# caishiqing/voice-tts

Measured on AMD Instinct MI355X. Metric: audio_seconds_per_second, higher is better.
Workload: dtype bf16

## Files before the change

### voice-tts_amd/csrc/gemm_x6.hip

```cpp
#include "common.h"

namespace ixtts {

typedef float gx_f32x16 __attribute__((ext_vector_type(16)));
typedef __bf16 gx_bf16x8 __attribute__((ext_vector_type(8)));
typedef float gx_f32x4 __attribute__((ext_vector_type(4)));
typedef unsigned int gx_u32x4 __attribute__((ext_vector_type(4)));


__global__ void gemm_x6_pack_kernel(const float* __restrict__ w, uint4* __restrict__ out, int N, int K, int Npad) {
  const long total = (long)(K / 8) * Npad;
  for (long idx = blockIdx.x * (long)blockDim.x + threadIdx.x; idx < total; idx += (long)gridDim.x * blockDim.x) {
    const int n = (int)(idx % Npad);
    const int ko = (int)(idx / Npad);
    float v[8];
#pragma unroll
    for (int e = 0; e < 8; ++e) v[e] = n < N ? w[(long)n * K + ko * 8 + e] : 0.f;
    uint4 ph, pm, pl;
    split8_bf16x3(v, ph, pm, pl);
    const int g = ko >> 1, kh = ko & 1;
    uint4* base = out + ((long)g * 6) * Npad + n;
    base[(long)(0 * 2 + kh) * Npad] = ph;
    base[(long)(1 * 2 + kh) * Npad] = pm;
    base[(long)(2 * 2 + kh) * Npad] = pl;
  }
}

template <int HALO>
__device__ __forceinline__ long split_src_row(long rr, int hT, int hleft, int hright, const int* __restrict__ hoff, int hn) {
  if constexpr (HALO == 0) return rr;
  long o0;
  int T = hT;
  if constexpr (HALO == 1) {
    o0 = rr / (hleft + hT + hright) * (hleft + hT + hright);
  } else {
    const int s = seq_of_row(hoff, hn, rr);
    o0 = hoff[s];
    T = hoff[s + 1] - (int)o0 - hleft - hright;
    if (T <= hleft || T <= hright) return rr;
  }
  const int h = (int)(rr - o0);
  if (h < hleft) return o0 + 2 * hleft - h;
  if (h >= hleft + T && h < hleft + T + hright) return o0 + 2 * (hleft + T) - 2 - h;
  return rr;
}

template <int HALO = 0>
__global__ __launch_bounds__(256) void gemm_x6_split_kernel(const float* __restrict__ a, long lda, uint4* __restrict__ out, int M, int K, long Mpad, int hT = 0,
                                                            int hleft = 0, int hright = 0, const int* __restrict__ hoff = nullptr, int hn = 0) {
  __shared__ float tile[64][65];
  const int r0 = blockIdx.x * 64, k0 = blockIdx.y * 64;
  const int t = threadIdx.x;
#pragma unroll
  for (int i = 0; i < 4; ++i) {
    const int r = (t >> 4) + 16 * i, kq = t & 15;
    float4 v = make_float4(0.f, 0.f, 0.f, 0.f);
    if (r0 + r < M) v = *reinterpret_cast<const float4*>(a + split_src_row<HALO>(r0 + r, hT, hleft, hright, hoff, hn) * lda + k0 + 4 * kq);
    tile[r][4 * kq + 0] = v.x; tile[r][4 * kq + 1] = v.y; tile[r][4 * kq + 2] = v.z; tile[r][4 * kq + 3] = v.w;
  }
  __syncthreads();
#pragma unroll
  for (int u = 0; u < 2; ++u) {
    const int r = t & 63, o = (t >> 6) + 4 * u;
    float v[8];
#pragma unroll
    for (int e = 0; e < 8; ++e) v[e] = tile[r][o * 8 + e];
    uint4 ph, pm, pl;
    split8_bf16x3(v, ph, pm, pl);
    const int ko = (k0 >> 3) + o, g = ko >> 1, kh = ko & 1;
    uint4* base = out + ((long)g * 6) * Mpad + r0 + r;
    base[(long)(0 * 2 + kh) * Mpad] = ph;
    base[(long)(1 * 2 + kh) * Mpad] = pm;
    base[(long)(2 * 2 + kh) * Mpad] = pl;
  }
}

enum { EPI_PLAIN = 0, EPI_SWIGLU = 1, EPI_GATE = 2 };

struct GemmX6Params {
  const uint4* Ap;
  long Mpad;
  long arow0;
  const uint4* Wp;
  const float* bias;
  float* C;
  long ldc;
  int M, N, Npad, K, accumulate, m_tiles, n_tiles;
  int tap_steps;
  int epi;
  const float* gate;
  long gate_ld, rows_per_batch;
  int nbatch;
  const int* gate_seq_off;
  unsigned long long* dbg;
};


template <int MT, int NT, int NST, int EPI = EPI_PLAIN, int ACC = 0, int SEQ = 0, int DBG = 0, int PIN = 0>
__global__ __launch_bounds__(256, (NST * (MT + NT) * 6 * 64 * 16 <= 80 * 1024) ? 2 : 1) void gemm_x6_kernel(GemmX6Params p) {
  constexpr int BM = 64 * MT, BN = 64 * NT;
  constexpr int A_UNITS = 6 * BM, W_UNITS = 6 * BN, STAGE = A_UNITS + W_UNITS;
  constexpr int NDMA = (6 * (MT + NT)) / 4;
  constexpr int NA = (6 * MT) / 4, NW = NDMA - NA;
  static_assert((6 * MT) % 4 == 0 && (6 * NT) % 4 == 0, "the A pieces and the W pieces are each dealt evenly to the 4 waves");
  static_assert(EPI == EPI_PLAIN || (ACC == 0 && NT == 2), "pair epilogues: the wave's two 32-column blocks are the two halves");
  static_assert(EPI == EPI_GATE || SEQ == 0, "the sequence table belongs to the gate epilogue");
  constexpr int D = NST - 1;
  extern __shared__ uint4 smem[];

  const int nwg = p.m_tiles * p.n_tiles;
  const int bid = blockIdx.x;
  const int xcd = bid & 7, idx = bid >> 3;
  const int qd = nwg >> 3, rm = nwg & 7;
  const int lin = (xcd < rm ? xcd * (qd + 1) : rm * (qd + 1) + (xcd - rm) * qd) + idx;
  const int m_tile = lin / p.n_tiles, n_tile = lin - m_tile * p.n_tiles;
  const int m0 = m_tile * BM, n0 = n_tile * BN;

  const int tid = threadIdx.x, lane = tid & 63;
  const int wave = __builtin_amdgcn_readfirstlane(tid >> 6);
  const int wm = wave >> 1, wn = wave & 1;
  const int l31 = lane & 31, lh = lane >> 5;

  gx_f32x16 acc[MT][NT];
#pragma unroll
  for (int i = 0; i < MT; ++i)
#pragma unroll
    for (int j = 0; j < NT; ++j)
#pragma unroll
      for (int r = 0; r < 16; ++r) acc[i][j][r] = 0.f;

  const uint4* asrc = p.Ap + p.arow0 + m0 + lane;
  const uint4* wsrc = p.Wp + n0 + lane;
  long a_off[NA], w_off[NW];
  int a_lds[NA], w_lds[NW];
#pragma unroll
  for (int q = 0; q < NA; ++q) {
    const int e = q * 4 + wave, run = e / MT, piece = e % MT;
    a_off[q] = run * p.Mpad + piece * 64;
    a_lds[q] = run * BM + piece * 64;
  }
#pragma unroll
  for (int q = 0; q < NW; ++q) {
    const int e = q * 4 + wave, run = e / NT, piece = e % NT;
    w_off[q] = (long)run * p.Npad + piece * 64;
    w_lds[q] = A_UNITS + run * BN + piece * 64;
  }
  const long a_step = 6 * p.Mpad, w_step = 6L * p.Npad;
  const long a_wrap = 1 - p.tap_steps * a_step;
  long a_run = 0, w_run = 0;
  int a_group = 0;
  auto issue_next = [&](uint4* st) {
#pragma unroll
    for (int q = 0; q < NA; ++q)
      __builtin_amdgcn_global_load_lds((const __attribute__((address_space(1))) void*)(asrc + (a_off[q] + a_run)),
                                       (__attribute__((address_space(3))) void*)(st + a_lds[q]), 16, 0, 0);
#pragma unroll
    for (int q = 0; q < NW; ++q)
      __builtin_amdgcn_global_load_lds((const __attribute__((address_space(1))) void*)(wsrc + (w_off[q] + w_run)),
                                       (__attribute__((address_space(3))) void*)(st + w_lds[q]), 16, 0, 0);
    a_run += a_step;
    w_run += w_step;
    if (++a_group == p.tap_steps) {
      a_group = 0;
      a_run += a_wrap;
    }
  };

  const int steps = p.K >> 4;
  auto wg_stamp = [&](int k) {
    if constexpr (DBG == 3) {
      if (tid == 0) p.dbg[128 + (long)blockIdx.x * 4 + k] = __builtin_amdgcn_s_memrealtime();
    }
  };
  auto wait_younger = [&](int y) {
    if (y >= 2) asm volatile("s_waitcnt vmcnt(%0)" ::"n"(2 * NDMA) : "memory");
    else if (y == 1) asm volatile("s_waitcnt vmcnt(%0)" ::"n"(NDMA) : "memory");
    else asm volatile("s_waitcnt vmcnt(0)" ::: "memory");
  };
  static_assert(D >= 1 && D <= 3, "1..3 steps of copies in flight behind the one waited for");
  wg_stamp(0);
  for (int t = 0; t < D && t < steps; ++t) issue_next(smem + t * STAGE);
  wait_younger(min(D, steps) - 1);
  __builtin_amdgcn_s_barrier();
  asm volatile("" ::: "memory");
  wg_stamp(1);

  const unsigned base_addr = (unsigned)(uintptr_t)(const __attribute__((address_space(3))) void*)smem;
  int st_cur = 0, st_nxt = D % NST;
  for (int s = 0; s < steps; ++s) {
    auto stamp = [&](int k) {
      if constexpr (DBG == 3) {
        if (blockIdx.x == 0 && tid == 0 && s < 16) {
          p.dbg[s * 8 + k] = __builtin_amdgcn_s_memtime();
          if (k == 0) p.dbg[s * 8 + 7] = __builtin_amdgcn_s_memrealtime();
        }
      }
    };
    stamp(0);
    if (DBG != 1 && s + D < steps) issue_next(smem + st_nxt * STAGE);
    stamp(1);
    const unsigned cur_addr = base_addr + (unsigned)(st_cur * STAGE * 16);
    if constexpr (DBG != 2) {
      gx_u32x4 af[3][MT], bf[3][NT];
      const unsigned aaddr = cur_addr + (unsigned)((lh * BM + wm * (32 * MT) + l31) * 16);
      const unsigned waddr = cur_addr + (unsigned)((A_UNITS + lh * BN + wn * (32 * NT) + l31) * 16);
      if constexpr (MT == 4 && NT == 2) {
        asm volatile(
            "ds_read_b128 %0, %18 offset:%20\n ds_read_b128 %1, %18 offset:%21\n ds_read_b128 %2, %18 offset:%22\n ds_read_b128 %3, %18 offset:%23\n"
            "ds_read_b128 %4, %18 offset:%24\n ds_read_b128 %5, %18 offset:%25\n ds_read_b128 %6, %18 offset:%26\n ds_read_b128 %7, %18 offset:%27\n"
            "ds_read_b128 %8, %18 offset:%28\n ds_read_b128 %9, %18 offset:%29\n ds_read_b128 %10, %18 offset:%30\n ds_read_b128 %11, %18 offset:%31\n"
            "ds_read_b128 %12, %19 offset:%32\n ds_read_b128 %13, %19 offset:%33\n ds_read_b128 %14, %19 offset:%34\n ds_read_b128 %15, %19 offset:%35\n"
            "ds_read_b128 %16, %19 offset:%36\n ds_read_b128 %17, %19 offset:%37\n s_waitcnt lgkmcnt(0)"
            : "=&v"(af[0][0]), "=&v"(af[0][1]), "=&v"(af[0][2]), "=&v"(af[0][3]), "=&v"(af[1][0]), "=&v"(af[1][1]), "=&v"(af[1][2]), "=&v"(af[1][3]),
              "=&v"(af[2][0]), "=&v"(af[2][1]), "=&v"(af[2][2]), "=&v"(af[2][3]), "=&v"(bf[0][0]), "=&v"(bf[0][1]), "=&v"(bf[1][0]), "=&v"(bf[1][1]),
              "=&v"(bf[2][0]), "=&v"(bf[2][1])
            : "v"(aaddr), "v"(waddr), "n"((0 * 2 * BM + 0) * 16), "n"((0 * 2 * BM + 32) * 16), "n"((0 * 2 * BM + 64) * 16), "n"((0 * 2 * BM + 96) * 16),
              "n"((1 * 2 * BM + 0) * 16), "n"((1 * 2 * BM + 32) * 16), "n"((1 * 2 * BM + 64) * 16), "n"((1 * 2 * BM + 96) * 16), "n"((2 * 2 * BM + 0) * 16),
              "n"((2 * 2 * BM + 32) * 16), "n"((2 * 2 * BM + 64) * 16), "n"((2 * 2 * BM + 96) * 16), "n"((0 * 2 * BN + 0) * 16), "n"((0 * 2 * BN + 32) * 16),
              "n"((1 * 2 * BN + 0) * 16), "n"((1 * 2 * BN + 32) * 16), "n"((2 * 2 * BN + 0) * 16), "n"((2 * 2 * BN + 32) * 16)
            : "memory");
      } else {
        static_assert(MT == 2 && NT == 2, "fragment block written for 256 x 128 and 128 x 128 tiles");
        asm volatile(
            "ds_read_b128 %0, %12 offset:%14\n ds_read_b128 %1, %12 offset:%15\n ds_read_b128 %2, %12 offset:%16\n ds_read_b128 %3, %12 offset:%17\n"
            "ds_read_b128 %4, %12 offset:%18\n ds_read_b128 %5, %12 offset:%19\n ds_read_b128 %6, %13 offset:%20\n ds_read_b128 %7, %13 offset:%21\n"
            "ds_read_b128 %8, %13 offset:%22\n ds_read_b128 %9, %13 offset:%23\n ds_read_b128 %10, %13 offset:%24\n ds_read_b128 %11, %13 offset:%25\n"
            "s_waitcnt lgkmcnt(0)"
            : "=&v"(af[0][0]), "=&v"(af[0][1]), "=&v"(af[1][0]), "=&v"(af[1][1]), "=&v"(af[2][0]), "=&v"(af[2][1]), "=&v"(bf[0][0]), "=&v"(bf[0][1]),
              "=&v"(bf[1][0]), "=&v"(bf[1][1]), "=&v"(bf[2][0]), "=&v"(bf[2][1])
            : "v"(aaddr), "v"(waddr), "n"((0 * 2 * BM + 0) * 16), "n"((0 * 2 * BM + 32) * 16), "n"((1 * 2 * BM + 0) * 16), "n"((1 * 2 * BM + 32) * 16),
              "n"((2 * 2 * BM + 0) * 16), "n"((2 * 2 * BM + 32) * 16), "n"((0 * 2 * BN + 0) * 16), "n"((0 * 2 * BN + 32) * 16), "n"((1 * 2 * BN + 0) * 16),
              "n"((1 * 2 * BN + 32) * 16), "n"((2 * 2 * BN + 0) * 16), "n"((2 * 2 * BN + 32) * 16)
            : "memory");
      }
      stamp(2);
#pragma unroll
      for (int i = 0; i < MT; ++i)
#pragma unroll
        for (int j = 0; j < NT; ++j) {
          const gx_bf16x8 ah = __builtin_bit_cast(gx_bf16x8, af[0][i]), am = __builtin_bit_cast(gx_bf16x8, af[1][i]), al = __builtin_bit_cast(gx_bf16x8, af[2][i]);
          const gx_bf16x8 bh = __builtin_bit_cast(gx_bf16x8, bf[0][j]), bm = __builtin_bit_cast(gx_bf16x8, bf[1][j]), bl = __builtin_bit_cast(gx_bf16x8, bf[2][j]);
          acc[i][j] = __builtin_amdgcn_mfma_f32_32x32x16_bf16(al, bh, acc[i][j], 0, 0, 0);
          acc[i][j] = __builtin_amdgcn_mfma_f32_32x32x16_bf16(ah, bl, acc[i][j], 0, 0, 0);
          acc[i][j] = __builtin_amdgcn_mfma_f32_32x32x16_bf16(am, bm, acc[i][j], 0, 0, 0);
          acc[i][j] = __builtin_amdgcn_mfma_f32_32x32x16_bf16(am, bh, acc[i][j], 0, 0, 0);
          acc[i][j] = __builtin_amdgcn_mfma_f32_32x32x16_bf16(ah, bm, acc[i][j], 0, 0, 0);
          acc[i][j] = __builtin_amdgcn_mfma_f32_32x32x16_bf16(ah, bh, acc[i][j], 0, 0, 0);
        }
      if constexpr (DBG == 3) asm volatile("" ::"v"(acc[0][0][0]), "v"(acc[MT - 1][NT - 1][15]));
      if constexpr (PIN != 0) __builtin_amdgcn_sched_barrier(0);
    }
    stamp(3);
    wait_younger(DBG == 1 ? 0 : max(0, min(D - 1, steps - s - 2)));
    stamp(4);
    __builtin_amdgcn_s_barrier();
    asm volatile("" ::: "memory");
    stamp(5);
    st_cur = st_cur + 1 == NST ? 0 : st_cur + 1;
    st_nxt = st_nxt + 1 == NST ? 0 : st_nxt + 1;
  }

  wg_stamp(2);
  if constexpr (EPI != EPI_PLAIN) {
    const int oc = (n0 + wn * 64) / 2 + l31;
    const int nh = p.N >> 1;
    if (oc < nh) {
      const unsigned rpb = (unsigned)min(p.rows_per_batch, (long)0x7fffffff);
      const float ba = p.bias != nullptr ? p.bias[n0 + wn * 64 + l31] : 0.f, bb = p.bias != nullptr ? p.bias[n0 + wn * 64 + 32 + l31] : 0.f;
#pragma unroll
      for (int i = 0; i < MT; ++i) {
        const int rbase = m0 + wm * (32 * MT) + i * 32 + 4 * lh;
#pragma unroll
        for (int r = 0; r < 16; ++r) {
          const int row = rbase + (r & 3) + 8 * (r >> 2);
          if (row < p.M) {
            float a = acc[i][0][r] + ba, b = acc[i][1][r] + bb, v;
            if constexpr (EPI == EPI_SWIGLU) {
              v = a / (1.0f + expf(-a)) * b;
            } else {
              long gb;
              if constexpr (SEQ != 0) gb = (long)seq_of_row(p.gate_seq_off, p.nbatch, row);
              else gb = min((long)((unsigned)row / rpb), (long)p.nbatch - 1);
              const float* g = p.gate + gb * p.gate_ld;
              a += g[oc];
              b += g[nh + oc];
              v = tanhf(a) * (1.0f / (1.0f + expf(-b)));
            }
            p.C[(long)row * p.ldc + oc] = v;
          }
        }
      }
    }
  } else
#pragma unroll
  for (int j = 0; j < NT; ++j) {
    const int col = n0 + wn * (32 * NT) + j * 32 + l31;
    const bool col_ok = col < p.N;
    const float bv = (p.bias != nullptr && col_ok) ? p.bias[col] : 0.f;
#pragma unroll
    for (int i = 0; i < MT; ++i) {
      const int rbase = m0 + wm * (32 * MT) + i * 32 + 4 * lh;
#pragma unroll
      for (int r = 0; r < 16; ++r) {
        const int row = rbase + (r & 3) + 8 * (r >> 2);
        if (col_ok && row < p.M) {
          float* c = p.C + (long)row * p.ldc + col;
          float v = acc[i][j][r] + bv;
          if constexpr (ACC != 0) v += *c;
          *c = v;
        }
      }
    }
  }
  if constexpr (DBG == 3) {
    asm volatile("s_waitcnt vmcnt(0)" ::: "memory");
    wg_stamp(3);
  }
}

template <int MT, int NT, int NST, int EPI = EPI_PLAIN, int ACC = 0, int SEQ = 0, int DBG = 0, int PIN = 0>
static int launch_gemm_x6(GemmX6Params p, hipStream_t st) {
  constexpr int BM = 64 * MT, BN = 64 * NT;
  constexpr size_t smem = (size_t)NST * (6 * BM + 6 * BN) * 16;
  static_assert(smem <= 160 * 1024, "LDS stages of this tile shape");
  p.m_tiles = ceil_div(p.M, BM);
  p.n_tiles = ceil_div(p.N, BN);
  IX_ARG((long)p.n_tiles * BN <= p.Npad, "gemm_x6: packed weights padded to %d features, the %d-wide tile needs %d", p.Npad, BN, p.n_tiles * BN);
  const int taps = (p.K >> 4) / p.tap_steps;
  IX_ARG(p.arow0 + (long)p.m_tiles * BM + taps - 1 <= p.Mpad, "gemm_x6: activation planes hold %ld rows, the %d-row tiles reach row %ld", p.Mpad, BM,
         p.arow0 + (long)p.m_tiles * BM + taps - 1);
  auto kern = gemm_x6_kernel<MT, NT, NST, EPI, ACC, SEQ, DBG, PIN>;
  static bool done = false;
  if (!done) {
    IX_HIP(hipFuncSetAttribute((const void*)kern, hipFuncAttributeMaxDynamicSharedMemorySize, (int)smem));
    done = true;
  }
  hipLaunchKernelGGL(kern, dim3(p.m_tiles * p.n_tiles), dim3(256), smem, st, p);
  IX_HIP(hipGetLastError());
  return IXTTS_OK;
}

template <int MT, int NT, int NST, bool PAIR>
static int launch_gemm_x6_epilogue(const GemmX6Params& p, hipStream_t st) {
  if (p.epi == EPI_PLAIN) return p.accumulate ? launch_gemm_x6<MT, NT, NST, EPI_PLAIN, 1>(p, st) : launch_gemm_x6<MT, NT, NST, EPI_PLAIN, 0>(p, st);
  if constexpr (PAIR) {
    if (p.epi == EPI_SWIGLU) return launch_gemm_x6<MT, NT, NST, EPI_SWIGLU>(p, st);
    if (p.epi == EPI_GATE)
      return p.gate_seq_off ? launch_gemm_x6<MT, NT, NST, EPI_GATE, 0, 1>(p, st) : launch_gemm_x6<MT, NT, NST, EPI_GATE, 0, 0>(p, st);
  }
  set_error("gemm_x6: epilogue %d on a tile shape built without it", p.epi);
  return IXTTS_ERR_ARG;
}

}

using namespace ixtts;

extern "C" size_t ixtts_gemm_x6_packed_bytes(int N, int K) {
  if (N <= 0 || K <= 0 || K % 64) return 0;
  const size_t Npad = (size_t)(N + 255) / 256 * 256;
  return (size_t)(K / 16) * 6 * Npad * 16;
}

extern "C" int ixtts_gemm_x6_pack(const float* w_dev, void* packed_dev, int N, int K, void* stream) {
  IX_ARG(w_dev && packed_dev && N > 0 && K > 0 && K % 64 == 0, "gemm_x6_pack: bad argument (K must be a multiple of 64)");
  const int Npad = (N + 255) / 256 * 256;
  const long total = (long)(K / 8) * Npad;
  hipLaunchKernelGGL(gemm_x6_pack_kernel, dim3((unsigned)std::min<long>((total + 255) / 256, 4096)), dim3(256), 0, (hipStream_t)stream, w_dev,
                     reinterpret_cast<uint4*>(packed_dev), N, K, Npad);
  IX_HIP(hipGetLastError());
  return IXTTS_OK;
}

extern "C" long ixtts_gemm_x6_rows_padded(long rows) { return rows <= 0 ? 0 : (rows + 255) / 256 * 256 + 256; }

extern "C" int ixtts_gemm_x6_split(const float* a_dev, long lda, void* planes_dev, long rows, int K, void* stream) {
  IX_ARG(a_dev && planes_dev && rows > 0 && K > 0 && K % 64 == 0, "gemm_x6_split: bad argument (K must be a multiple of 64)");
  IX_ARG(lda >= K && lda % 4 == 0 && (reinterpret_cast<uintptr_t>(a_dev) & 15) == 0, "gemm_x6_split: rows must be 16-byte aligned (lda %ld)", lda);
  const long Mpad = ixtts_gemm_x6_rows_padded(rows);
  hipLaunchKernelGGL(gemm_x6_split_kernel<0>, dim3((unsigned)(Mpad / 64), K / 64), dim3(256), 0, (hipStream_t)stream, a_dev, lda,
                     reinterpret_cast<uint4*>(planes_dev), (int)rows, K, Mpad);
  IX_HIP(hipGetLastError());
  return IXTTS_OK;
}

extern "C" int ixtts_gemm_x6_split_halo(const float* a_dev, long lda, void* planes_dev, long rows, int K, int T, int left, int right, void* stream) {
  IX_ARG(a_dev && planes_dev && rows > 0 && K > 0 && K % 64 == 0, "gemm_x6_split_halo: bad argument (K must be a multiple of 64)");
  IX_ARG(lda >= K && lda % 4 == 0 && (reinterpret_cast<uintptr_t>(a_dev) & 15) == 0, "gemm_x6_split_halo: rows must be 16-byte aligned (lda %ld)", lda);
  IX_ARG(left >= 0 && right >= 0 && T > left && T > right && rows % (left + T + right) == 0,
         "gemm_x6_split_halo: bad shape rows=%ld T=%d left=%d right=%d (rows = whole sequences of left + T + right)", rows, T, left, right);
  const long Mpad = ixtts_gemm_x6_rows_padded(rows);
  hipLaunchKernelGGL(gemm_x6_split_kernel<1>, dim3((unsigned)(Mpad / 64), K / 64), dim3(256), 0, (hipStream_t)stream, a_dev, lda,
                     reinterpret_cast<uint4*>(planes_dev), (int)rows, K, Mpad, T, left, right);
  IX_HIP(hipGetLastError());
  return IXTTS_OK;
}

extern "C" int ixtts_gemm_x6_split_halo_varlen(const float* a_dev, long lda, void* planes_dev, long rows, int K, const int* seq_off_dev, int nseq, int left,
                                               int right, void* stream) {
  IX_ARG(a_dev && planes_dev && seq_off_dev && rows > 0 && K > 0 && K % 64 == 0, "gemm_x6_split_halo_varlen: bad argument (K must be a multiple of 64)");
  IX_ARG(lda >= K && lda % 4 == 0 && (reinterpret_cast<uintptr_t>(a_dev) & 15) == 0, "gemm_x6_split_halo_varlen: rows must be 16-byte aligned (lda %ld)", lda);
  IX_ARG(nseq > 0 && left >= 0 && right >= 0, "gemm_x6_split_halo_varlen: bad shape nseq=%d left=%d right=%d", nseq, left, right);
  const long Mpad = ixtts_gemm_x6_rows_padded(rows);
  hipLaunchKernelGGL(gemm_x6_split_kernel<2>, dim3((unsigned)(Mpad / 64), K / 64), dim3(256), 0, (hipStream_t)stream, a_dev, lda,
                     reinterpret_cast<uint4*>(planes_dev), (int)rows, K, Mpad, 0, left, right, seq_off_dev, nseq);
  IX_HIP(hipGetLastError());
  return IXTTS_OK;
}

static int run_gemm_x6(GemmX6Params p, int tile, hipStream_t st) {
  if (tile == 0) {
    const long t42 = (long)ceil_div(p.M, 256) * ceil_div(p.N, 128);
    tile = t42 >= 140 ? 2 : 3;
  }
  switch (tile) {
    case 2: return launch_gemm_x6_epilogue<4, 2, 2, true>(p, st);
    case 3: return launch_gemm_x6_epilogue<2, 2, 3, true>(p, st);
    case 4: return launch_gemm_x6_epilogue<4, 2, 4, false>(p, st);
    case 5: return launch_gemm_x6_epilogue<2, 2, 4, false>(p, st);
  }
  if (tile >= 12 && (p.epi != EPI_PLAIN || p.accumulate)) {
    set_error("gemm_x6: the developer variants (tile %d) are built with the plain, overwriting epilogue only", tile);
    return IXTTS_ERR_ARG;
  }
  switch (tile) {
    case 12: return launch_gemm_x6<4, 2, 2, EPI_PLAIN, 0, 0, 1>(p, st);
    case 22: return launch_gemm_x6<4, 2, 2, EPI_PLAIN, 0, 0, 2>(p, st);
    case 32: return launch_gemm_x6<4, 2, 2, EPI_PLAIN, 0, 0, 3>(p, st);
    case 33: return launch_gemm_x6<2, 2, 3, EPI_PLAIN, 0, 0, 3>(p, st);
    case 42: return launch_gemm_x6<4, 2, 2, EPI_PLAIN, 0, 0, 0, 1>(p, st);
    case 43: return launch_gemm_x6<2, 2, 3, EPI_PLAIN, 0, 0, 0, 1>(p, st);
  }
  set_error("gemm_x6: tile %d (0 auto; 2 / 3: 256x128 / 128x128, two workgroups per CU; 4 / 5: the same, one per CU with a 4-stage ring)", tile);
  return IXTTS_ERR_ARG;
}

extern "C" int ixtts_gemm_x6_f32(const void* a_planes_dev, long rows_total, long row0, const void* packed_dev, const float* bias_dev, float* c_dev,
                                 long ldc, int M, int N, int K, int accumulate, int tile, void* stream) {
  IX_ARG(a_planes_dev && packed_dev && c_dev && M > 0 && N > 0 && K > 0 && K % 64 == 0, "gemm_x6: bad argument (K must be a multiple of 64: the split pass works on 64-wide k blocks)");
  IX_ARG(ldc >= N && row0 >= 0 && row0 + M <= rows_total, "gemm_x6: rows [%ld, %ld) of %ld, ldc %ld", row0, row0 + M, rows_total, ldc);
  GemmX6Params p;
  p.Ap = reinterpret_cast<const uint4*>(a_planes_dev); p.Mpad = ixtts_gemm_x6_rows_padded(rows_total); p.arow0 = row0;
  p.Wp = reinterpret_cast<const uint4*>(packed_dev); p.bias = bias_dev; p.C = c_dev; p.ldc = ldc;
  p.M = M; p.N = N; p.Npad = (N + 255) / 256 * 256; p.K = K; p.accumulate = accumulate ? 1 : 0; p.m_tiles = p.n_tiles = 0;
  p.tap_steps = K >> 4; p.epi = EPI_PLAIN; p.gate = nullptr; p.gate_ld = 0; p.rows_per_batch = 1; p.nbatch = 1; p.gate_seq_off = nullptr;
  p.dbg = (tile == 32 || tile == 33) ? reinterpret_cast<unsigned long long*>(const_cast<float*>(bias_dev)) : nullptr;
  if (p.dbg) p.bias = nullptr;
  return run_gemm_x6(p, tile, (hipStream_t)stream);
}

extern "C" int ixtts_gemm_x6_pair_f32(const void* a_planes_dev, long rows_total, long row0, int taps, const void* packed_dev, const float* bias_dev,
                                      const float* gate_dev, long gate_ld, long rows_per_batch, int nbatch, float* c_dev, long ldc, int M, int N, int K,
                                      int epilogue, int tile, void* stream) {
  IX_ARG(a_planes_dev && packed_dev && c_dev && M > 0 && N > 0 && taps > 0 && K > 0, "gemm_x6_pair: bad argument");
  IX_ARG(K % taps == 0 && (K / taps) % 64 == 0 && N % 64 == 0, "gemm_x6_pair: K %d = %d taps of a multiple of 64, N %d a multiple of 64", K, taps, N);
  IX_ARG(epilogue == EPI_SWIGLU || (epilogue == EPI_GATE && gate_dev && rows_per_batch > 0 && nbatch > 0 && gate_ld >= N / 2),
         "gemm_x6_pair: epilogue %d (1 swiglu; 2 gate, with gate biases)", epilogue);
  IX_ARG(ldc >= N / 2 && row0 >= 0 && row0 + M + taps - 1 <= rows_total, "gemm_x6_pair: rows [%ld, %ld) + %d taps of %ld, ldc %ld", row0, row0 + M, taps,
         rows_total, ldc);
  IX_ARG(tile == 0 || tile == 2 || tile == 3, "gemm_x6_pair: tile %d (0 auto, 2, 3)", tile);
  GemmX6Params p;
  p.Ap = reinterpret_cast<const uint4*>(a_planes_dev); p.Mpad = ixtts_gemm_x6_rows_padded(rows_total); p.arow0 = row0;
  p.Wp = reinterpret_cast<const uint4*>(packed_dev); p.bias = bias_dev; p.C = c_dev; p.ldc = ldc;
  p.M = M; p.N = N; p.Npad = (N + 255) / 256 * 256; p.K = K; p.accumulate = 0; p.m_tiles = p.n_tiles = 0;
  p.tap_steps = (K / taps) >> 4; p.epi = epilogue; p.gate = gate_dev; p.gate_ld = gate_ld; p.rows_per_batch = rows_per_batch; p.nbatch = nbatch;
  p.gate_seq_off = nullptr;
  p.dbg = nullptr;
  return run_gemm_x6(p, tile, (hipStream_t)stream);
}

extern "C" int ixtts_gemm_x6_pair_gate_varlen_f32(const void* a_planes_dev, long rows_total, long row0, int taps, const void* packed_dev, const float* bias_dev,
                                                  const float* gate_dev, long gate_ld, const int* seq_off_dev, int nseq, float* c_dev, long ldc, int M, int N,
                                                  int K, int tile, void* stream) {
  IX_ARG(seq_off_dev && nseq > 0, "gemm_x6_pair_gate_varlen: null offsets table or nseq %d", nseq);
  IX_ARG(a_planes_dev && packed_dev && c_dev && gate_dev && M > 0 && N > 0 && taps > 0 && K > 0 && gate_ld >= N / 2, "gemm_x6_pair_gate_varlen: bad argument");
  IX_ARG(K % taps == 0 && (K / taps) % 64 == 0 && N % 64 == 0, "gemm_x6_pair_gate_varlen: K %d = %d taps of a multiple of 64, N %d a multiple of 64", K, taps, N);
  IX_ARG(ldc >= N / 2 && row0 >= 0 && row0 + M + taps - 1 <= rows_total, "gemm_x6_pair_gate_varlen: rows [%ld, %ld) + %d taps of %ld, ldc %ld", row0, row0 + M,
         taps, rows_total, ldc);
  IX_ARG(tile == 0 || tile == 2 || tile == 3, "gemm_x6_pair_gate_varlen: tile %d (0 auto, 2, 3)", tile);
  GemmX6Params p;
  p.Ap = reinterpret_cast<const uint4*>(a_planes_dev); p.Mpad = ixtts_gemm_x6_rows_padded(rows_total); p.arow0 = row0;
  p.Wp = reinterpret_cast<const uint4*>(packed_dev); p.bias = bias_dev; p.C = c_dev; p.ldc = ldc;
  p.M = M; p.N = N; p.Npad = (N + 255) / 256 * 256; p.K = K; p.accumulate = 0; p.m_tiles = p.n_tiles = 0;
  p.tap_steps = (K / taps) >> 4; p.epi = EPI_GATE; p.gate = gate_dev; p.gate_ld = gate_ld; p.rows_per_batch = 1; p.nbatch = nseq;
  p.gate_seq_off = seq_off_dev;
  p.dbg = nullptr;
  return run_gemm_x6(p, tile, (hipStream_t)stream);
}
```

Measured before the change: 41.73.

## Add software-pipelined 128x128 gemm_x6 loop interleaving LDS reads and copies with MFMAs

Adds a PIPE variant of the 6-MFMA split-bf16 GEMM kernel for 128x128 tiles with a 4-stage ring. It double-buffers register fragments so the next step's LDS reads and the global-to-LDS copies are issued among the current step's MFMAs, pinned in place with sched_barriers. The auto tile selection uses this variant when the 128x128 grid fits within the CU count, aiming to hide LDS and global latency in small, latency-bound GEMMs. The cost is more registers, one workgroup per CU, and a K%64 requirement.

```diff
diff --git a/voice-tts_amd/csrc/gemm_x6.hip b/voice-tts_amd/csrc/gemm_x6.hip
--- a/voice-tts_amd/csrc/gemm_x6.hip
+++ b/voice-tts_amd/csrc/gemm_x6.hip
@@ -96,7 +96,7 @@
 };
 
 
-template <int MT, int NT, int NST, int EPI = EPI_PLAIN, int ACC = 0, int SEQ = 0, int DBG = 0, int PIN = 0>
+template <int MT, int NT, int NST, int EPI = EPI_PLAIN, int ACC = 0, int SEQ = 0, int DBG = 0, int PIN = 0, int PIPE = 0>
 __global__ __launch_bounds__(256, (NST * (MT + NT) * 6 * 64 * 16 <= 80 * 1024) ? 2 : 1) void gemm_x6_kernel(GemmX6Params p) {
   constexpr int BM = 64 * MT, BN = 64 * NT;
   constexpr int A_UNITS = 6 * BM, W_UNITS = 6 * BN, STAGE = A_UNITS + W_UNITS;
@@ -149,21 +149,26 @@
   const long a_wrap = 1 - p.tap_steps * a_step;
   long a_run = 0, w_run = 0;
   int a_group = 0;
-  auto issue_next = [&](uint4* st) {
-#pragma unroll
-    for (int q = 0; q < NA; ++q)
+  auto issue_piece = [&](uint4* st, int q) {
+    if (q < NA)
       __builtin_amdgcn_global_load_lds((const __attribute__((address_space(1))) void*)(asrc + (a_off[q] + a_run)),
                                        (__attribute__((address_space(3))) void*)(st + a_lds[q]), 16, 0, 0);
-#pragma unroll
-    for (int q = 0; q < NW; ++q)
-      __builtin_amdgcn_global_load_lds((const __attribute__((address_space(1))) void*)(wsrc + (w_off[q] + w_run)),
-                                       (__attribute__((address_space(3))) void*)(st + w_lds[q]), 16, 0, 0);
+    else
+      __builtin_amdgcn_global_load_lds((const __attribute__((address_space(1))) void*)(wsrc + (w_off[q - NA] + w_run)),
+                                       (__attribute__((address_space(3))) void*)(st + w_lds[q - NA]), 16, 0, 0);
+  };
+  auto issue_advance = [&]() {
     a_run += a_step;
     w_run += w_step;
     if (++a_group == p.tap_steps) {
       a_group = 0;
       a_run += a_wrap;
     }
+  };
+  auto issue_next = [&](uint4* st) {
+#pragma unroll
+    for (int q = 0; q < NDMA; ++q) issue_piece(st, q);
+    issue_advance();
   };
 
   const int steps = p.K >> 4;
@@ -179,16 +184,35 @@
   };
   static_assert(D >= 1 && D <= 3, "1..3 steps of copies in flight behind the one waited for");
   wg_stamp(0);
-  for (int t = 0; t < D && t < steps; ++t) issue_next(smem + t * STAGE);
-  wait_younger(min(D, steps) - 1);
-  __builtin_amdgcn_s_barrier();
-  asm volatile("" ::: "memory");
-  wg_stamp(1);
-
-  const unsigned base_addr = (unsigned)(uintptr_t)(const __attribute__((address_space(3))) void*)smem;
-  int st_cur = 0, st_nxt = D % NST;
-  for (int s = 0; s < steps; ++s) {
-    auto stamp = [&](int k) {
+  if constexpr (PIPE != 0) {
+    static_assert(MT == 2 && NT == 2 && NST == 4 && PIN == 0 && (DBG == 0 || DBG == 3), "the pipelined loop: 128 x 128 tile, 4 stages");
+    static_assert(D % NST != 0 && D % NST != 1 % NST && D % NST != 2 % NST, "(b): the copy target is none of the stages of steps s, s + 1, s + 2");
+    constexpr int RD_AT = 1, CP_AT = 2, CP_EVERY = 3;
+    static_assert(RD_AT < CP_AT && CP_AT + (NDMA - 1) * CP_EVERY < 6 * MT * NT, "reads, then the copies, all among the step's MFMAs");
+    const unsigned base_addr = (unsigned)(uintptr_t)(const __attribute__((address_space(3))) void*)smem;
+    const unsigned a_rel = (unsigned)((lh * BM + wm * (32 * MT) + l31) * 16), w_rel = (unsigned)((A_UNITS + lh * BN + wn * (32 * NT) + l31) * 16);
+    gx_u32x4 fa[2][3][MT], fb[2][3][NT];
+    auto read_issue = [&](gx_u32x4 (&a)[3][MT], gx_u32x4 (&b)[3][NT], int stage) {
+      const unsigned aaddr = base_addr + (unsigned)(stage * STAGE * 16) + a_rel, waddr = base_addr + (unsigned)(stage * STAGE * 16) + w_rel;
+      asm volatile(
+          "ds_read_b128 %0, %12 offset:%14\n ds_read_b128 %1, %12 offset:%15\n ds_read_b128 %2, %12 offset:%16\n ds_read_b128 %3, %12 offset:%17\n"
+          "ds_read_b128 %4, %12 offset:%18\n ds_read_b128 %5, %12 offset:%19\n ds_read_b128 %6, %13 offset:%20\n ds_read_b128 %7, %13 offset:%21\n"
+          "ds_read_b128 %8, %13 offset:%22\n ds_read_b128 %9, %13 offset:%23\n ds_read_b128 %10, %13 offset:%24\n ds_read_b128 %11, %13 offset:%25"
+          : "=&v"(a[0][0]), "=&v"(a[0][1]), "=&v"(a[1][0]), "=&v"(a[1][1]), "=&v"(a[2][0]), "=&v"(a[2][1]), "=&v"(b[0][0]),
+            "=&v"(b[0][1]), "=&v"(b[1][0]), "=&v"(b[1][1]), "=&v"(b[2][0]), "=&v"(b[2][1])
+          : "v"(aaddr), "v"(waddr), "n"((0 * 2 * BM + 0) * 16), "n"((0 * 2 * BM + 32) * 16), "n"((1 * 2 * BM + 0) * 16), "n"((1 * 2 * BM + 32) * 16),
+            "n"((2 * 2 * BM + 0) * 16), "n"((2 * 2 * BM + 32) * 16), "n"((0 * 2 * BN + 0) * 16), "n"((0 * 2 * BN + 32) * 16), "n"((1 * 2 * BN + 0) * 16),
+            "n"((1 * 2 * BN + 32) * 16), "n"((2 * 2 * BN + 0) * 16), "n"((2 * 2 * BN + 32) * 16)
+          : "memory");
+    };
+    auto read_wait = [&](gx_u32x4 (&a)[3][MT], gx_u32x4 (&b)[3][NT]) {
+      asm volatile("s_waitcnt lgkmcnt(0)"
+                   : "+v"(a[0][0]), "+v"(a[0][1]), "+v"(a[1][0]), "+v"(a[1][1]), "+v"(a[2][0]), "+v"(a[2][1]), "+v"(b[0][0]),
+                     "+v"(b[0][1]), "+v"(b[1][0]), "+v"(b[1][1]), "+v"(b[2][0]), "+v"(b[2][1])
+                   :
+                   : "memory");
+    };
+    auto stamp = [&](int s, int k) {
       if constexpr (DBG == 3) {
         if (blockIdx.x == 0 && tid == 0 && s < 16) {
           p.dbg[s * 8 + k] = __builtin_amdgcn_s_memtime();
@@ -196,68 +220,166 @@
         }
       }
     };
-    stamp(0);
-    if (DBG != 1 && s + D < steps) issue_next(smem + st_nxt * STAGE);
-    stamp(1);
-    const unsigned cur_addr = base_addr + (unsigned)(st_cur * STAGE * 16);
-    if constexpr (DBG != 2) {
-      gx_u32x4 af[3][MT], bf[3][NT];
-      const unsigned aaddr = cur_addr + (unsigned)((lh * BM + wm * (32 * MT) + l31) * 16);
-      const unsigned waddr = cur_addr + (unsigned)((A_UNITS + lh * BN + wn * (32 * NT) + l31) * 16);
-      if constexpr (MT == 4 && NT == 2) {
-        asm volatile(
-            "ds_read_b128 %0, %18 offset:%20\n ds_read_b128 %1, %18 offset:%21\n ds_read_b128 %2, %18 offset:%22\n ds_read_b128 %3, %18 offset:%23\n"
-            "ds_read_b128 %4, %18 offset:%24\n ds_read_b128 %5, %18 offset:%25\n ds_read_b128 %6, %18 offset:%26\n ds_read_b128 %7, %18 offset:%27\n"
-            "ds_read_b128 %8, %18 offset:%28\n ds_read_b128 %9, %18 offset:%29\n ds_read_b128 %10, %18 offset:%30\n ds_read_b128 %11, %18 offset:%31\n"
-            "ds_read_b128 %12, %19 offset:%32\n ds_read_b128 %13, %19 offset:%33\n ds_read_b128 %14, %19 offset:%34\n ds_read_b128 %15, %19 offset:%35\n"
-            "ds_read_b128 %16, %19 offset:%36\n ds_read_b128 %17, %19 offset:%37\n s_waitcnt lgkmcnt(0)"
-            : "=&v"(af[0][0]), "=&v"(af[0][1]), "=&v"(af[0][2]), "=&v"(af[0][3]), "=&v"(af[1][0]), "=&v"(af[1][1]), "=&v"(af[1][2]), "=&v"(af[1][3]),
-              "=&v"(af[2][0]), "=&v"(af[2][1]), "=&v"(af[2][2]), "=&v"(af[2][3]), "=&v"(bf[0][0]), "=&v"(bf[0][1]), "=&v"(bf[1][0]), "=&v"(bf[1][1]),
-              "=&v"(bf[2][0]), "=&v"(bf[2][1])
-            : "v"(aaddr), "v"(waddr), "n"((0 * 2 * BM + 0) * 16), "n"((0 * 2 * BM + 32) * 16), "n"((0 * 2 * BM + 64) * 16), "n"((0 * 2 * BM + 96) * 16),
-              "n"((1 * 2 * BM + 0) * 16), "n"((1 * 2 * BM + 32) * 16), "n"((1 * 2 * BM + 64) * 16), "n"((1 * 2 * BM + 96) * 16), "n"((2 * 2 * BM + 0) * 16),
-              "n"((2 * 2 * BM + 32) * 16), "n"((2 * 2 * BM + 64) * 16), "n"((2 * 2 * BM + 96) * 16), "n"((0 * 2 * BN + 0) * 16), "n"((0 * 2 * BN + 32) * 16),
-              "n"((1 * 2 * BN + 0) * 16), "n"((1 * 2 * BN + 32) * 16), "n"((2 * 2 * BN + 0) * 16), "n"((2 * 2 * BN + 32) * 16)
-            : "memory");
+    int st_rd = 1, st_cp = D % NST;
+    auto step = [&](auto set, auto copy, auto read, auto sync, int s) {
+      constexpr int c = decltype(set)::value;
+      constexpr bool COPY = decltype(copy)::value, READ = decltype(read)::value, SYNC = decltype(sync)::value;
+      static_assert(READ || !COPY, "copies are only issued for steps that will be read");
+      static_assert(READ || !SYNC, "the closing wait and barrier publish data to a later read block");
+      stamp(s, 0);
+      if constexpr (DBG == 3) __builtin_amdgcn_sched_barrier(0);
+      uint4* const cp_stage = smem + st_cp * STAGE;
+      auto among = [&](int k) {
+        if (READ && k == RD_AT) {
+          __builtin_amdgcn_sched_barrier(0);
+          read_issue(fa[1 - c], fb[1 - c], st_rd);
+          __builtin_amdgcn_sched_barrier(0);
+        }
+        if (COPY && k >= CP_AT && (k - CP_AT) % CP_EVERY == 0 && (k - CP_AT) / CP_EVERY < NDMA) {
+          __builtin_amdgcn_sched_barrier(0);
+          issue_piece(cp_stage, (k - CP_AT) / CP_EVERY);
+          __builtin_amdgcn_sched_barrier(0);
+        }
+      };
+#pragma unroll
+      for (int i = 0; i < MT; ++i)
+#pragma unroll
+        for (int j = 0; j < NT; ++j) {
+          const gx_bf16x8 ah = __builtin_bit_cast(gx_bf16x8, fa[c][0][i]), am = __builtin_bit_cast(gx_bf16x8, fa[c][1][i]), al = __builtin_bit_cast(gx_bf16x8, fa[c][2][i]);
+          const gx_bf16x8 bh = __builtin_bit_cast(gx_bf16x8, fb[c][0][j]), bm = __builtin_bit_cast(gx_bf16x8, fb[c][1][j]), bl = __builtin_bit_cast(gx_bf16x8, fb[c][2][j]);
+          const int k0 = (i * NT + j) * 6;
+          acc[i][j] = __builtin_amdgcn_mfma_f32_32x32x16_bf16(al, bh, acc[i][j], 0, 0, 0);
+          among(k0 + 0);
+          acc[i][j] = __builtin_amdgcn_mfma_f32_32x32x16_bf16(ah, bl, acc[i][j], 0, 0, 0);
+          among(k0 + 1);
+          acc[i][j] = __builtin_amdgcn_mfma_f32_32x32x16_bf16(am, bm, acc[i][j], 0, 0, 0);
+          among(k0 + 2);
+          acc[i][j] = __builtin_amdgcn_mfma_f32_32x32x16_bf16(am, bh, acc[i][j], 0, 0, 0);
+          among(k0 + 3);
+          acc[i][j] = __builtin_amdgcn_mfma_f32_32x32x16_bf16(ah, bm, acc[i][j], 0, 0, 0);
+          among(k0 + 4);
+          acc[i][j] = __builtin_amdgcn_mfma_f32_32x32x16_bf16(ah, bh, acc[i][j], 0, 0, 0);
+          among(k0 + 5);
+        }
+      if constexpr (COPY) issue_advance();
+      if constexpr (DBG == 3) asm volatile("" ::"v"(acc[0][0][0]), "v"(acc[MT - 1][NT - 1][15]));
+      stamp(s, 1);
+      if constexpr (READ) read_wait(fa[1 - c], fb[1 - c]);
+      stamp(s, 2);
+      if constexpr (SYNC) {
+        wait_younger(COPY ? 1 : 0);
+        stamp(s, 3);
+        __builtin_amdgcn_s_barrier();
+        asm volatile("" ::: "memory");
       } else {
-        static_assert(MT == 2 && NT == 2, "fragment block written for 256 x 128 and 128 x 128 tiles");
-        asm volatile(
-            "ds_read_b128 %0, %12 offset:%14\n ds_read_b128 %1, %12 offset:%15\n ds_read_b128 %2, %12 offset:%16\n ds_read_b128 %3, %12 offset:%17\n"
-            "ds_read_b128 %4, %12 offset:%18\n ds_read_b128 %5, %12 offset:%19\n ds_read_b128 %6, %13 offset:%20\n ds_read_b128 %7, %13 offset:%21\n"
-            "ds_read_b128 %8, %13 offset:%22\n ds_read_b128 %9, %13 offset:%23\n ds_read_b128 %10, %13 offset:%24\n ds_read_b128 %11, %13 offset:%25\n"
-            "s_waitcnt lgkmcnt(0)"
-            : "=&v"(af[0][0]), "=&v"(af[0][1]), "=&v"(af[1][0]), "=&v"(af[1][1]), "=&v"(af[2][0]), "=&v"(af[2][1]), "=&v"(bf[0][0]), "=&v"(bf[0][1]),
-              "=&v"(bf[1][0]), "=&v"(bf[1][1]), "=&v"(bf[2][0]), "=&v"(bf[2][1])
-            : "v"(aaddr), "v"(waddr), "n"((0 * 2 * BM + 0) * 16), "n"((0 * 2 * BM + 32) * 16), "n"((1 * 2 * BM + 0) * 16), "n"((1 * 2 * BM + 32) * 16),
-              "n"((2 * 2 * BM + 0) * 16), "n"((2 * 2 * BM + 32) * 16), "n"((0 * 2 * BN + 0) * 16), "n"((0 * 2 * BN + 32) * 16), "n"((1 * 2 * BN + 0) * 16),
-              "n"((1 * 2 * BN + 32) * 16), "n"((2 * 2 * BN + 0) * 16), "n"((2 * 2 * BN + 32) * 16)
-            : "memory");
+        stamp(s, 3);
       }
-      stamp(2);
-#pragma unroll
-      for (int i = 0; i < MT; ++i)
-#pragma unroll
-        for (int j = 0; j < NT; ++j) {
-          const gx_bf16x8 ah = __builtin_bit_cast(gx_bf16x8, af[0][i]), am = __builtin_bit_cast(gx_bf16x8, af[1][i]), al = __builtin_bit_cast(gx_bf16x8, af[2][i]);
-          const gx_bf16x8 bh = __builtin_bit_cast(gx_bf16x8, bf[0][j]), bm = __builtin_bit_cast(gx_bf16x8, bf[1][j]), bl = __builtin_bit_cast(gx_bf16x8, bf[2][j]);
-          acc[i][j] = __builtin_amdgcn_mfma_f32_32x32x16_bf16(al, bh, acc[i][j], 0, 0, 0);
-          acc[i][j] = __builtin_amdgcn_mfma_f32_32x32x16_bf16(ah, bl, acc[i][j], 0, 0, 0);
-          acc[i][j] = __builtin_amdgcn_mfma_f32_32x32x16_bf16(am, bm, acc[i][j], 0, 0, 0);
-          acc[i][j] = __builtin_amdgcn_mfma_f32_32x32x16_bf16(am, bh, acc[i][j], 0, 0, 0);
-          acc[i][j] = __builtin_amdgcn_mfma_f32_32x32x16_bf16(ah, bm, acc[i][j], 0, 0, 0);
-          acc[i][j] = __builtin_amdgcn_mfma_f32_32x32x16_bf16(ah, bh, acc[i][j], 0, 0, 0);
-        }
-      if constexpr (DBG == 3) asm volatile("" ::"v"(acc[0][0][0]), "v"(acc[MT - 1][NT - 1][15]));
-      if constexpr (PIN != 0) __builtin_amdgcn_sched_barrier(0);
-    }
-    stamp(3);
-    wait_younger(DBG == 1 ? 0 : max(0, min(D - 1, steps - s - 2)));
-    stamp(4);
+      stamp(s, 4);
+      st_rd = (st_rd + 1) & (NST - 1);
+      st_cp = (st_cp + 1) & (NST - 1);
+    };
+    constexpr std::integral_constant<int, 0> S0;
+    constexpr std::integral_constant<int, 1> S1;
+    constexpr std::true_type Y;
+    constexpr std::false_type N_;
+
+    for (int t = 0; t < D; ++t) issue_next(smem + t * STAGE);
+    wait_younger(1);
     __builtin_amdgcn_s_barrier();
     asm volatile("" ::: "memory");
-    stamp(5);
-    st_cur = st_cur + 1 == NST ? 0 : st_cur + 1;
-    st_nxt = st_nxt + 1 == NST ? 0 : st_nxt + 1;
+    read_issue(fa[0], fb[0], 0);
+    read_wait(fa[0], fb[0]);
+    wg_stamp(1);
+    int s = 0;
+    for (; s + 4 < steps; s += 2) {
+      step(S0, Y, Y, Y, s);
+      step(S1, Y, Y, Y, s + 1);
+    }
+    step(S0, Y, Y, Y, s);
+    step(S1, N_, Y, Y, s + 1);
+    step(S0, N_, Y, N_, s + 2);
+    step(S1, N_, N_, N_, s + 3);
+  } else {
+    for (int t = 0; t < D && t < steps; ++t) issue_next(smem + t * STAGE);
+    wait_younger(min(D, steps) - 1);
+    __builtin_amdgcn_s_barrier();
+    asm volatile("" ::: "memory");
+    wg_stamp(1);
+
+    const unsigned base_addr = (unsigned)(uintptr_t)(const __attribute__((address_space(3))) void*)smem;
+    int st_cur = 0, st_nxt = D % NST;
+    for (int s = 0; s < steps; ++s) {
+      auto stamp = [&](int k) {
+        if constexpr (DBG == 3) {
+          if (blockIdx.x == 0 && tid == 0 && s < 16) {
+            p.dbg[s * 8 + k] = __builtin_amdgcn_s_memtime();
+            if (k == 0) p.dbg[s * 8 + 7] = __builtin_amdgcn_s_memrealtime();
+          }
+        }
+      };
+      stamp(0);
+      if (DBG != 1 && s + D < steps) issue_next(smem + st_nxt * STAGE);
+      stamp(1);
+      const unsigned cur_addr = base_addr + (unsigned)(st_cur * STAGE * 16);
+      if constexpr (DBG != 2) {
+        gx_u32x4 af[3][MT], bf[3][NT];
+        const unsigned aaddr = cur_addr + (unsigned)((lh * BM + wm * (32 * MT) + l31) * 16);
+        const unsigned waddr = cur_addr + (unsigned)((A_UNITS + lh * BN + wn * (32 * NT) + l31) * 16);
+        if constexpr (MT == 4 && NT == 2) {
+          asm volatile(
+              "ds_read_b128 %0, %18 offset:%20\n ds_read_b128 %1, %18 offset:%21\n ds_read_b128 %2, %18 offset:%22\n ds_read_b128 %3, %18 offset:%23\n"
+              "ds_read_b128 %4, %18 offset:%24\n ds_read_b128 %5, %18 offset:%25\n ds_read_b128 %6, %18 offset:%26\n ds_read_b128 %7, %18 offset:%27\n"
+              "ds_read_b128 %8, %18 offset:%28\n ds_read_b128 %9, %18 offset:%29\n ds_read_b128 %10, %18 offset:%30\n ds_read_b128 %11, %18 offset:%31\n"
+              "ds_read_b128 %12, %19 offset:%32\n ds_read_b128 %13, %19 offset:%33\n ds_read_b128 %14, %19 offset:%34\n ds_read_b128 %15, %19 offset:%35\n"
+              "ds_read_b128 %16, %19 offset:%36\n ds_read_b128 %17, %19 offset:%37\n s_waitcnt lgkmcnt(0)"
+              : "=&v"(af[0][0]), "=&v"(af[0][1]), "=&v"(af[0][2]), "=&v"(af[0][3]), "=&v"(af[1][0]), "=&v"(af[1][1]), "=&v"(af[1][2]), "=&v"(af[1][3]),
+                "=&v"(af[2][0]), "=&v"(af[2][1]), "=&v"(af[2][2]), "=&v"(af[2][3]), "=&v"(bf[0][0]), "=&v"(bf[0][1]), "=&v"(bf[1][0]), "=&v"(bf[1][1]),
+                "=&v"(bf[2][0]), "=&v"(bf[2][1])
+              : "v"(aaddr), "v"(waddr), "n"((0 * 2 * BM + 0) * 16), "n"((0 * 2 * BM + 32) * 16), "n"((0 * 2 * BM + 64) * 16), "n"((0 * 2 * BM + 96) * 16),
+                "n"((1 * 2 * BM + 0) * 16), "n"((1 * 2 * BM + 32) * 16), "n"((1 * 2 * BM + 64) * 16), "n"((1 * 2 * BM + 96) * 16), "n"((2 * 2 * BM + 0) * 16),
+                "n"((2 * 2 * BM + 32) * 16), "n"((2 * 2 * BM + 64) * 16), "n"((2 * 2 * BM + 96) * 16), "n"((0 * 2 * BN + 0) * 16), "n"((0 * 2 * BN + 32) * 16),
+                "n"((1 * 2 * BN + 0) * 16), "n"((1 * 2 * BN + 32) * 16), "n"((2 * 2 * BN + 0) * 16), "n"((2 * 2 * BN + 32) * 16)
+              : "memory");
+        } else {
+          static_assert(MT == 2 && NT == 2, "fragment block written for 256 x 128 and 128 x 128 tiles");
+          asm volatile(
+              "ds_read_b128 %0, %12 offset:%14\n ds_read_b128 %1, %12 offset:%15\n ds_read_b128 %2, %12 offset:%16\n ds_read_b128 %3, %12 offset:%17\n"
+              "ds_read_b128 %4, %12 offset:%18\n ds_read_b128 %5, %12 offset:%19\n ds_read_b128 %6, %13 offset:%20\n ds_read_b128 %7, %13 offset:%21\n"
+              "ds_read_b128 %8, %13 offset:%22\n ds_read_b128 %9, %13 offset:%23\n ds_read_b128 %10, %13 offset:%24\n ds_read_b128 %11, %13 offset:%25\n"
+              "s_waitcnt lgkmcnt(0)"
+              : "=&v"(af[0][0]), "=&v"(af[0][1]), "=&v"(af[1][0]), "=&v"(af[1][1]), "=&v"(af[2][0]), "=&v"(af[2][1]), "=&v"(bf[0][0]), "=&v"(bf[0][1]),
+                "=&v"(bf[1][0]), "=&v"(bf[1][1]), "=&v"(bf[2][0]), "=&v"(bf[2][1])
+              : "v"(aaddr), "v"(waddr), "n"((0 * 2 * BM + 0) * 16), "n"((0 * 2 * BM + 32) * 16), "n"((1 * 2 * BM + 0) * 16), "n"((1 * 2 * BM + 32) * 16),
+                "n"((2 * 2 * BM + 0) * 16), "n"((2 * 2 * BM + 32) * 16), "n"((0 * 2 * BN + 0) * 16), "n"((0 * 2 * BN + 32) * 16), "n"((1 * 2 * BN + 0) * 16),
+                "n"((1 * 2 * BN + 32) * 16), "n"((2 * 2 * BN + 0) * 16), "n"((2 * 2 * BN + 32) * 16)
+              : "memory");
+        }
+        stamp(2);
+#pragma unroll
+        for (int i = 0; i < MT; ++i)
+#pragma unroll
+          for (int j = 0; j < NT; ++j) {
+            const gx_bf16x8 ah = __builtin_bit_cast(gx_bf16x8, af[0][i]), am = __builtin_bit_cast(gx_bf16x8, af[1][i]), al = __builtin_bit_cast(gx_bf16x8, af[2][i]);
+            const gx_bf16x8 bh = __builtin_bit_cast(gx_bf16x8, bf[0][j]), bm = __builtin_bit_cast(gx_bf16x8, bf[1][j]), bl = __builtin_bit_cast(gx_bf16x8, bf[2][j]);
+            acc[i][j] = __builtin_amdgcn_mfma_f32_32x32x16_bf16(al, bh, acc[i][j], 0, 0, 0);
+            acc[i][j] = __builtin_amdgcn_mfma_f32_32x32x16_bf16(ah, bl, acc[i][j], 0, 0, 0);
+            acc[i][j] = __builtin_amdgcn_mfma_f32_32x32x16_bf16(am, bm, acc[i][j], 0, 0, 0);
+            acc[i][j] = __builtin_amdgcn_mfma_f32_32x32x16_bf16(am, bh, acc[i][j], 0, 0, 0);
+            acc[i][j] = __builtin_amdgcn_mfma_f32_32x32x16_bf16(ah, bm, acc[i][j], 0, 0, 0);
+            acc[i][j] = __builtin_amdgcn_mfma_f32_32x32x16_bf16(ah, bh, acc[i][j], 0, 0, 0);
+          }
+        if constexpr (DBG == 3) asm volatile("" ::"v"(acc[0][0][0]), "v"(acc[MT - 1][NT - 1][15]));
+        if constexpr (PIN != 0) __builtin_amdgcn_sched_barrier(0);
+      }
+      stamp(3);
+      wait_younger(DBG == 1 ? 0 : max(0, min(D - 1, steps - s - 2)));
+      stamp(4);
+      __builtin_amdgcn_s_barrier();
+      asm volatile("" ::: "memory");
+      stamp(5);
+      st_cur = st_cur + 1 == NST ? 0 : st_cur + 1;
+      st_nxt = st_nxt + 1 == NST ? 0 : st_nxt + 1;
+    }
   }
 
   wg_stamp(2);
@@ -318,7 +440,7 @@
   }
 }
 
-template <int MT, int NT, int NST, int EPI = EPI_PLAIN, int ACC = 0, int SEQ = 0, int DBG = 0, int PIN = 0>
+template <int MT, int NT, int NST, int EPI = EPI_PLAIN, int ACC = 0, int SEQ = 0, int DBG = 0, int PIN = 0, int PIPE = 0>
 static int launch_gemm_x6(GemmX6Params p, hipStream_t st) {
   constexpr int BM = 64 * MT, BN = 64 * NT;
   constexpr size_t smem = (size_t)NST * (6 * BM + 6 * BN) * 16;
@@ -326,10 +448,11 @@
   p.m_tiles = ceil_div(p.M, BM);
   p.n_tiles = ceil_div(p.N, BN);
   IX_ARG((long)p.n_tiles * BN <= p.Npad, "gemm_x6: packed weights padded to %d features, the %d-wide tile needs %d", p.Npad, BN, p.n_tiles * BN);
+  if constexpr (PIPE != 0) IX_ARG(p.K > 0 && p.K % 64 == 0, "gemm_x6: the pipelined loop takes its steps in fours, K %d", p.K);
   const int taps = (p.K >> 4) / p.tap_steps;
   IX_ARG(p.arow0 + (long)p.m_tiles * BM + taps - 1 <= p.Mpad, "gemm_x6: activation planes hold %ld rows, the %d-row tiles reach row %ld", p.Mpad, BM,
          p.arow0 + (long)p.m_tiles * BM + taps - 1);
-  auto kern = gemm_x6_kernel<MT, NT, NST, EPI, ACC, SEQ, DBG, PIN>;
+  auto kern = gemm_x6_kernel<MT, NT, NST, EPI, ACC, SEQ, DBG, PIN, PIPE>;
   static bool done = false;
   if (!done) {
     IX_HIP(hipFuncSetAttribute((const void*)kern, hipFuncAttributeMaxDynamicSharedMemorySize, (int)smem));
@@ -340,13 +463,14 @@
   return IXTTS_OK;
 }
 
-template <int MT, int NT, int NST, bool PAIR>
+template <int MT, int NT, int NST, bool PAIR, int PIPE = 0>
 static int launch_gemm_x6_epilogue(const GemmX6Params& p, hipStream_t st) {
-  if (p.epi == EPI_PLAIN) return p.accumulate ? launch_gemm_x6<MT, NT, NST, EPI_PLAIN, 1>(p, st) : launch_gemm_x6<MT, NT, NST, EPI_PLAIN, 0>(p, st);
+  if (p.epi == EPI_PLAIN)
+    return p.accumulate ? launch_gemm_x6<MT, NT, NST, EPI_PLAIN, 1, 0, 0, 0, PIPE>(p, st) : launch_gemm_x6<MT, NT, NST, EPI_PLAIN, 0, 0, 0, 0, PIPE>(p, st);
   if constexpr (PAIR) {
-    if (p.epi == EPI_SWIGLU) return launch_gemm_x6<MT, NT, NST, EPI_SWIGLU>(p, st);
+    if (p.epi == EPI_SWIGLU) return launch_gemm_x6<MT, NT, NST, EPI_SWIGLU, 0, 0, 0, 0, PIPE>(p, st);
     if (p.epi == EPI_GATE)
-      return p.gate_seq_off ? launch_gemm_x6<MT, NT, NST, EPI_GATE, 0, 1>(p, st) : launch_gemm_x6<MT, NT, NST, EPI_GATE, 0, 0>(p, st);
+      return p.gate_seq_off ? launch_gemm_x6<MT, NT, NST, EPI_GATE, 0, 1, 0, 0, PIPE>(p, st) : launch_gemm_x6<MT, NT, NST, EPI_GATE, 0, 0, 0, 0, PIPE>(p, st);
   }
   set_error("gemm_x6: epilogue %d on a tile shape built without it", p.epi);
   return IXTTS_ERR_ARG;
@@ -408,16 +532,27 @@
   return IXTTS_OK;
 }
 
+static long device_cu_count() {
+  static const long n = [] {
+    int dev = 0, cus = 0;
+    return (hipGetDevice(&dev) == hipSuccess && hipDeviceGetAttribute(&cus, hipDeviceAttributeMultiprocessorCount, dev) == hipSuccess) ? (long)cus : 0L;
+  }();
+  return n;
+}
+
 static int run_gemm_x6(GemmX6Params p, int tile, hipStream_t st) {
   if (tile == 0) {
     const long t42 = (long)ceil_div(p.M, 256) * ceil_div(p.N, 128);
     tile = t42 >= 140 ? 2 : 3;
+    static const bool pipe = !(getenv("IXTTS_GEMM_X6_PIPE") && !strcmp(getenv("IXTTS_GEMM_X6_PIPE"), "0"));
+    if (tile == 3 && pipe && (long)ceil_div(p.M, 128) * ceil_div(p.N, 128) <= device_cu_count()) tile = 6;
   }
   switch (tile) {
     case 2: return launch_gemm_x6_epilogue<4, 2, 2, true>(p, st);
     case 3: return launch_gemm_x6_epilogue<2, 2, 3, true>(p, st);
     case 4: return launch_gemm_x6_epilogue<4, 2, 4, false>(p, st);
     case 5: return launch_gemm_x6_epilogue<2, 2, 4, false>(p, st);
+    case 6: return launch_gemm_x6_epilogue<2, 2, 4, true, 1>(p, st);
   }
   if (tile >= 12 && (p.epi != EPI_PLAIN || p.accumulate)) {
     set_error("gemm_x6: the developer variants (tile %d) are built with the plain, overwriting epilogue only", tile);
@@ -428,10 +563,11 @@
     case 22: return launch_gemm_x6<4, 2, 2, EPI_PLAIN, 0, 0, 2>(p, st);
     case 32: return launch_gemm_x6<4, 2, 2, EPI_PLAIN, 0, 0, 3>(p, st);
     case 33: return launch_gemm_x6<2, 2, 3, EPI_PLAIN, 0, 0, 3>(p, st);
+    case 36: return launch_gemm_x6<2, 2, 4, EPI_PLAIN, 0, 0, 3, 0, 1>(p, st);
     case 42: return launch_gemm_x6<4, 2, 2, EPI_PLAIN, 0, 0, 0, 1>(p, st);
     case 43: return launch_gemm_x6<2, 2, 3, EPI_PLAIN, 0, 0, 0, 1>(p, st);
   }
-  set_error("gemm_x6: tile %d (0 auto; 2 / 3: 256x128 / 128x128, two workgroups per CU; 4 / 5: the same, one per CU with a 4-stage ring)", tile);
+  set_error("gemm_x6: tile %d (0 auto; 2 / 3: 256x128 / 128x128, two workgroups per CU; 4 / 5: the same, one per CU with a 4-stage ring; 6: 128x128, one per CU, pipelined loop)", tile);
   return IXTTS_ERR_ARG;
 }
 
@@ -444,7 +580,7 @@
   p.Wp = reinterpret_cast<const uint4*>(packed_dev); p.bias = bias_dev; p.C = c_dev; p.ldc = ldc;
   p.M = M; p.N = N; p.Npad = (N + 255) / 256 * 256; p.K = K; p.accumulate = accumulate ? 1 : 0; p.m_tiles = p.n_tiles = 0;
   p.tap_steps = K >> 4; p.epi = EPI_PLAIN; p.gate = nullptr; p.gate_ld = 0; p.rows_per_batch = 1; p.nbatch = 1; p.gate_seq_off = nullptr;
-  p.dbg = (tile == 32 || tile == 33) ? reinterpret_cast<unsigned long long*>(const_cast<float*>(bias_dev)) : nullptr;
+  p.dbg = (tile == 32 || tile == 33 || tile == 36) ? reinterpret_cast<unsigned long long*>(const_cast<float*>(bias_dev)) : nullptr;
   if (p.dbg) p.bias = nullptr;
   return run_gemm_x6(p, tile, (hipStream_t)stream);
 }
@@ -458,7 +594,7 @@
          "gemm_x6_pair: epilogue %d (1 swiglu; 2 gate, with gate biases)", epilogue);
   IX_ARG(ldc >= N / 2 && row0 >= 0 && row0 + M + taps - 1 <= rows_total, "gemm_x6_pair: rows [%ld, %ld) + %d taps of %ld, ldc %ld", row0, row0 + M, taps,
          rows_total, ldc);
-  IX_ARG(tile == 0 || tile == 2 || tile == 3, "gemm_x6_pair: tile %d (0 auto, 2, 3)", tile);
+  IX_ARG(tile == 0 || tile == 2 || tile == 3 || tile == 6, "gemm_x6_pair: tile %d (0 auto, 2, 3, 6)", tile);
   GemmX6Params p;
   p.Ap = reinterpret_cast<const uint4*>(a_planes_dev); p.Mpad = ixtts_gemm_x6_rows_padded(rows_total); p.arow0 = row0;
   p.Wp = reinterpret_cast<const uint4*>(packed_dev); p.bias = bias_dev; p.C = c_dev; p.ldc = ldc;
@@ -477,7 +613,7 @@
   IX_ARG(K % taps == 0 && (K / taps) % 64 == 0 && N % 64 == 0, "gemm_x6_pair_gate_varlen: K %d = %d taps of a multiple of 64, N %d a multiple of 64", K, taps, N);
   IX_ARG(ldc >= N / 2 && row0 >= 0 && row0 + M + taps - 1 <= rows_total, "gemm_x6_pair_gate_varlen: rows [%ld, %ld) + %d taps of %ld, ldc %ld", row0, row0 + M,
          taps, rows_total, ldc);
-  IX_ARG(tile == 0 || tile == 2 || tile == 3, "gemm_x6_pair_gate_varlen: tile %d (0 auto, 2, 3)", tile);
+  IX_ARG(tile == 0 || tile == 2 || tile == 3 || tile == 6, "gemm_x6_pair_gate_varlen: tile %d (0 auto, 2, 3, 6)", tile);
   GemmX6Params p;
   p.Ap = reinterpret_cast<const uint4*>(a_planes_dev); p.Mpad = ixtts_gemm_x6_rows_padded(rows_total); p.arow0 = row0;
   p.Wp = reinterpret_cast<const uint4*>(packed_dev); p.bias = bias_dev; p.C = c_dev; p.ldc = ldc;
```

New measurement: 42.18, median of 6. 1.01x the previous value.
